# davide-coccomini/MINTIME-Multi-Identity-size-iNvariant-TIMEsformer-for-Video-Deepfake-Detection

Measured on AMD Instinct MI355X. Metric: clips/sec (8-frame, 2-identity, 224^2 crops) fwd+bwd, higher is better.
Workload: dtype f32; 1 GPU; config 3: EfficientNet-B0 + SizeInvariantTimeSformer(dim 512, depth 9, heads 8), B=32/GPU, 8 frames, 2 identities (identity-masked), 224x224 crops, random-init seeded weights (restored before every step), train-mode BN + drop-connect 0.2, step = fwd + BCE loss + bwd + SGD(lr .01, wd 1e-4); global_batch=32, frames=8, parallelism=dp1

## Files before the change

mintime-multi-identity-size-invariant-timesformer-for-video-deepfake-detection_amd/csrc/common.hpp:

```cpp
#pragma once
#include <hip/hip_runtime.h>
#include <stdio.h>
#include <stdarg.h>
#include <stdlib.h>
#include <map>
#include <mutex>
#include <utility>

namespace mt {

inline char* err_buf() {
  static thread_local char buf[512] = {0};
  return buf;
}

inline int fail(int code, const char* fmt, ...) {
  va_list ap;
  va_start(ap, fmt);
  vsnprintf(err_buf(), 512, fmt, ap);
  va_end(ap);
  return code;
}

inline int env_int(const char* name, int dflt) {
  const char* e = getenv(name);
  return e ? atoi(e) : dflt;
}
inline bool env_set(const char* name) { return getenv(name) != nullptr; }

inline int cur_device() {
  int d = 0;
  (void)hipGetDevice(&d);
  return d & 15;
}

inline hipError_t ensure_dynamic_lds(const void* kernel, size_t bytes) {
  if (bytes <= 48 * 1024) return hipSuccess;
  static std::mutex mu;
  static std::map<std::pair<const void*, int>, size_t> raised;
  int dev = 0;
  (void)hipGetDevice(&dev);
  std::lock_guard<std::mutex> g(mu);
  size_t& r = raised[std::make_pair(kernel, dev)];
  if (bytes <= r) return hipSuccess;
  const hipError_t e = hipFuncSetAttribute(kernel, hipFuncAttributeMaxDynamicSharedMemorySize, (int)bytes);
  if (e == hipSuccess) r = bytes;
  return e;
}

inline int check_launch(const char* what) {
  hipError_t e = hipGetLastError();
  if (e != hipSuccess) return fail(-2, "%s: launch failed: %s", what, hipGetErrorString(e));
  return 0;
}

int stem_wgrad_mfma(const float* du, const float* z, const float* kabc, const void* x, int x_is_u8, float* dw, int N, int H, int W,
                    int Ho, int Wo, int pad0, hipStream_t st);

enum { MT_ERR_ARG = -1, MT_ERR_LAUNCH = -2, MT_ERR_UNSUPPORTED = -3 };

int matmul_precision();

__device__ __forceinline__ void stat_add(double* p, int64_t limb, float v) {
  if (limb == 0) {
    atomicAdd(p, (double)v);
    return;
  }
  const float t = truncf(v);
  atomicAdd(reinterpret_cast<unsigned long long*>(p), (unsigned long long)(long long)t);
  atomicAdd(reinterpret_cast<unsigned long long*>(p + limb), (unsigned long long)__float2ll_rn((v - t) * 17592186044416.0f));
}
__device__ __forceinline__ double stat_get(const double* p, int64_t limb) {
  if (limb == 0) return *p;
  const long long hi = *reinterpret_cast<const long long*>(p), lo = *reinterpret_cast<const long long*>(p + limb);
  return (double)hi + (double)lo * 5.684341886080801486968994140625e-14;
}
__host__ __device__ __forceinline__ int stat_slots(int slots) { return slots < 0 ? -slots : (slots > 0 ? slots : 1); }
__host__ __device__ __forceinline__ int64_t stat_limb(int slots, int C) { return slots < 0 ? (int64_t)(-slots) * 2 * C : 0; }

__device__ __forceinline__ void xcd_chunk_tile(int chunks, int& chunk, int64_t& tile0, int64_t& stride) {
  const int xcd = blockIdx.x & 7, j = blockIdx.x >> 3;
  chunk = j % chunks;
  tile0 = (int64_t)(j / chunks) * 8 + xcd;
  stride = (int64_t)((gridDim.x >> 3) / chunks) * 8;
}

__device__ __forceinline__ void tile_nyx(int64_t tile, int ty_n, int tx_n, int& n, int& ty, int& tx) {
  const unsigned t = (unsigned)tile, t2 = t / (unsigned)tx_n;
  tx = (int)(t - t2 * (unsigned)tx_n);
  const unsigned nn = t2 / (unsigned)ty_n;
  ty = (int)(t2 - nn * (unsigned)ty_n);
  n = (int)nn;
}

__device__ __forceinline__ int64_t div_rows(int64_t r, int hw) {
  return (r >> 32) ? r / hw : (int64_t)((unsigned)r / (unsigned)hw);
}

struct FastDiv {
  uint32_t mul;
  int sh;
  __device__ __forceinline__ int div(int n) const { return mul ? (int)(__umulhi((uint32_t)n, mul) >> sh) : n; }
};
inline FastDiv fast_div_of(int d) {
  FastDiv f{0u, 0};
  if (d <= 1) return f;
  int l = 0;
  while (((int64_t)1 << l) < d) ++l;
  f.mul = (uint32_t)((((uint64_t)1 << (31 + l)) / (uint64_t)d) + 1);
  f.sh = l - 1;
  return f;
}

inline unsigned xcd_chunk_grid(int chunks, int64_t ntiles, int target_blocks) {
  if (ntiles >= ((int64_t)1 << 31)) return 0;
  int64_t per_xcd = target_blocks / (8 * chunks);
  const int64_t need = (ntiles + 7) / 8;
  if (per_xcd > need) per_xcd = need;
  if (per_xcd < 1) per_xcd = 1;
  return (unsigned)(8 * chunks * per_xcd);
}


__device__ __forceinline__ void lds_barrier() { asm volatile("s_waitcnt lgkmcnt(0)\n\ts_barrier" ::: "memory"); }

}
```

mintime-multi-identity-size-invariant-timesformer-for-video-deepfake-detection_amd/csrc/effnet_bwd.hip:

```cpp
#include "../../include/mintime_hip.h"
#include "common.hpp"
#include <type_traits>
#include "rc.hpp"
#include "det.hpp"
#include <stdlib.h>

using namespace mt;

namespace {

__device__ __forceinline__ float sigmoidf_(float x) { return __builtin_amdgcn_rcpf(1.0f + __expf(-x)); }
__device__ __forceinline__ float swishf_(float x) { return x * sigmoidf_(x); }
__device__ __forceinline__ float dswishf_(float u) { const float s = sigmoidf_(u); return s * (1.0f + u * (1.0f - s)); }

__device__ __forceinline__ float4 f4(float a, float b, float c, float d) { return make_float4(a, b, c, d); }
__device__ __forceinline__ float4 ld4(const float* p) { return *reinterpret_cast<const float4*>(p); }
__device__ __forceinline__ void st4(float* p, float4 v) { *reinterpret_cast<float4*>(p) = v; }
__device__ __forceinline__ float4 fma4(float4 a, float4 b, float4 c) {
  return f4(fmaf(a.x, b.x, c.x), fmaf(a.y, b.y, c.y), fmaf(a.z, b.z, c.z), fmaf(a.w, b.w, c.w));
}
__device__ __forceinline__ float4 mul4(float4 a, float4 b) { return f4(a.x * b.x, a.y * b.y, a.z * b.z, a.w * b.w); }
__device__ __forceinline__ float4 add4(float4 a, float4 b) { return f4(a.x + b.x, a.y + b.y, a.z + b.z, a.w + b.w); }

template <int ACT>
// ... 298 lines not shown
  constexpr int P = S == 1 ? (K - 1) / 2 : (K - 2) / 2;
  constexpr int CQN = CC / 4;
  constexpr int IH = (T - 1) * S + K;
  constexpr int IWP = IH | 1;
  constexpr int PS = (256 / CQN) / K;
  extern __shared__ __attribute__((aligned(16))) float lds[];
  float* a_t = lds;
  float* dz_t = lds + IH * IWP * CC;
  const int tid = threadIdx.x;
  const int cq = tid % CQN, r = tid / CQN;
  const int kh = r % K, ps = r / K;
  const bool worker = ps < PS;
  int chunk_id; int64_t tile0, tile_stride;
  xcd_chunk_tile(C / CC, chunk_id, tile0, tile_stride);
  const int c0 = chunk_id * CC;
  const int ty_n = (Ho + T - 1) / T, tx_n = (Wo + T - 1) / T;
  const int64_t ntiles = (int64_t)N * ty_n * tx_n;

  const float4 ka = ld4(kabc + c0 + cq * 4), kb = ld4(kabc + C + c0 + cq * 4), kc = ld4(kabc + 2 * C + c0 + cq * 4);
  const int lane = tid & 63;
  const int f_q = RC ? (lane >> 4) : cq, f_slot = RC ? ((tid >> 6) * 16 + (lane & 15)) : tid / CQN;
  const float4 sc = ld4(scale_in + c0 + f_q * 4), sh = ld4(shift_in + c0 + f_q * 4);
  constexpr int RCW = RC ? RC : 8;
  RcFrag<RCW> wfrag;
  if constexpr (RC > 0) rc_load<RCW>(wfrag, we + (int64_t)(c0 + (lane & 15)) * RC, lane);

  float4 acc[K];
#pragma unroll
  for (int i = 0; i < K; ++i) acc[i] = f4(0, 0, 0, 0);

  constexpr int NSL = 256 / CQN;
  constexpr int NL = (IH * IH + NSL - 1) / NSL, ND = (T * T + NSL - 1) / NSL;
  static_assert(NL <= 32 && ND <= 32, "validity masks are 32 bits");
  const int slot = tid / CQN;
  float4 pre[RC ? 1 : NL], pdu[ND], pz[ND];
  RcFrag<RCW> ypre[RC ? NL : 1];
  unsigned pre_ok = 0, pd_ok = 0;
  auto fetch = [&](int64_t tile) {
    int n, ty, tx;
    tile_nyx(tile, ty_n, tx_n, n, ty, tx);
    const int oh0 = ty * T, ow0 = tx * T;
    const int ih0 = oh0 * S - P, iw0 = ow0 * S - P;
    const float* img = RC ? zin + (int64_t)n * H * W * RC : zin + (int64_t)n * H * W * C + c0 + cq * 4;
    pre_ok = 0; pd_ok = 0;
#pragma unroll
    for (int i = 0; i < NL; ++i) {
      const int pix = f_slot + i * NSL;
      const int iy = pix / IH, ix = pix - iy * IH;
      const int ih = ih0 + iy, iw = iw0 + ix;
      if (pix < IH * IH && ih >= 0 && ih < H && iw >= 0 && iw < W) pre_ok |= 1u << i;
      const int64_t poff = (int64_t)min(max(ih, 0), H - 1) * W + min(max(iw, 0), W - 1);
      if constexpr (RC > 0) rc_load<RCW>(ypre[i], img + poff * RC, lane);
      else pre[i] = ld4(img + poff * C);
    }
    const int64_t obase = (int64_t)n * Ho * Wo * C + c0 + cq * 4;
#pragma unroll
    for (int i = 0; i < ND; ++i) {
      const int pix = slot + i * NSL;
      const int oy = pix / T, ox = pix - oy * T;
      const int oh = oh0 + oy, ow = ow0 + ox;
      if (pix < T * T && oh < Ho && ow < Wo) pd_ok |= 1u << i;
      const int64_t off = obase + ((int64_t)min(oh, Ho - 1) * Wo + min(ow, Wo - 1)) * C;
      pdu[i] = ld4(du + off);
      pz[i] = ld4(z + off);
    }
  };
  int64_t tile = tile0;
  if (tile < ntiles) fetch(tile);
  for (; tile < ntiles; tile += tile_stride) {
    __syncthreads();
#pragma unroll
    for (int i = 0; i < NL; ++i) {
      const int pix = f_slot + i * NSL;
      float4 zraw;
      if constexpr (RC > 0) zraw = rc_mma<RCW>(wfrag, ypre[i]);
      else zraw = pre[i];
      if (pix < IH * IH) {
        const int iy = pix / IH, ix = pix - iy * IH;
        const float4 v = act4<ACT>(fma4(zraw, sc, sh));
        const bool ok = (pre_ok >> i) & 1u;
        st4(a_t + (iy * IWP + ix) * CC + f_q * 4, f4(ok ? v.x : 0.f, ok ? v.y : 0.f, ok ? v.z : 0.f, ok ? v.w : 0.f));
      }
    }
#pragma unroll
    for (int i = 0; i < ND; ++i) {
      const int pix = slot + i * NSL;
      if (pix < T * T) {
        const float4 v = fma4(ka, pdu[i], fma4(kb, pz[i], kc));
        const bool ok = (pd_ok >> i) & 1u;
        st4(dz_t + pix * CC + cq * 4, f4(ok ? v.x : 0.f, ok ? v.y : 0.f, ok ? v.z : 0.f, ok ? v.w : 0.f));
      }
    }
    __syncthreads();
    if (tile + tile_stride < ntiles) fetch(tile + tile_stride);
    if (worker) {
      for (int p = ps; p < T * T; p += PS) {
        const int oy = p / T, ox = p - oy * T;
        const float4 d = ld4(dz_t + p * CC + cq * 4);
        const float* arow = a_t + ((oy * S + kh) * IWP + ox * S) * CC + cq * 4;
#pragma unroll
        for (int kw = 0; kw < K; ++kw) acc[kw] = fma4(d, ld4(arow + kw * CC), acc[kw]);
      }
    }
  }
  __syncthreads();
  float* red = lds;
  if (worker) {
#pragma unroll
    for (int kw = 0; kw < K; ++kw) st4(red + (((ps * K + kh) * CQN + cq) * K + kw) * 4, acc[kw]);
  }
  __syncthreads();
  if (tid < K * CQN * K) {
    const int kw = tid % K, q = (tid / K) % CQN, khh = tid / (CQN * K);
    float4 t = f4(0, 0, 0, 0);
    for (int g = 0; g < PS; ++g) t = add4(t, ld4(red + (((g * K + khh) * CQN + q) * K + kw) * 4));
    const int c = c0 + q * 4, tp = khh * K + kw;
    if (det.vals) {
      const int rk = (int)tile0, jb = q * 4 * K * K + tp;
      det_put(det, chunk_id, rk, jb, t.x); det_put(det, chunk_id, rk, jb + K * K, t.y);
      det_put(det, chunk_id, rk, jb + 2 * K * K, t.z); det_put(det, chunk_id, rk, jb + 3 * K * K, t.w);
      if (rk == 0 && tid == 0) det_base(det, chunk_id, (int64_t)c0 * K * K);
    } else {
      atomicAdd(dw + (c + 0) * K * K + tp, t.x); atomicAdd(dw + (c + 1) * K * K + tp, t.y);
      atomicAdd(dw + (c + 2) * K * K + tp, t.z); atomicAdd(dw + (c + 3) * K * K + tp, t.w);
    }
  }
}

template <int K, int S, int T, int ACT, int CC, int RC = 0>
int launch_dw_wgrad_tiled(const float* du, const float* z, const float* kabc, const float* zin, const float* scale_in,
                          const float* shift_in, float* dw, int N, int H, int W, int C, int Ho, int Wo, hipStream_t s,
                          const float* we = nullptr) {
  constexpr int IH = (T - 1) * S + K;
  constexpr int IWP = IH | 1;
  constexpr int CQN = CC / 4;
  constexpr int PS = (256 / CQN) / K;
  size_t lds = (size_t)(IH * IWP * CC + T * T * CC) * sizeof(float);
  const size_t red = (size_t)PS * K * CQN * K * 4 * sizeof(float);
  if (red > lds) lds = red;
  const int chunks = C / CC;
  const int64_t ntiles = (int64_t)N * ((Ho + T - 1) / T) * ((Wo + T - 1) / T);
  const unsigned bx = xcd_chunk_grid(chunks, ntiles, 4096);
  auto k = dwconv_wgrad_tiled_kernel<K, S, T, ACT, CC, RC>;
  if (lds > 48 * 1024) {
    hipError_t e = ensure_dynamic_lds(reinterpret_cast<const void*>(k), lds);
    if (e != hipSuccess) return fail(MT_ERR_LAUNCH, "mt_dwconv_bwd: cannot reserve %zu B of LDS: %s", lds, hipGetErrorString(e));
  }
  DetScope det(s, chunks, (int)((bx >> 3) / chunks) * 8, CC * K * K);
  hipLaunchKernelGGL(k, dim3(bx), dim3(256), lds, s, du, z, kabc, zin, scale_in, shift_in, dw, N, H, W, C, Ho, Wo, det.log, we);
  const int rc = check_launch("mt_dwconv_bwd(weight, tiled)");
  return rc ? rc : det.reduce_f32(dw);
}

thread_local int g_res_stride = 1;

template <int K, int S, int T, int ACT, int CC, bool WG = false, int RC = 0>
__global__ __launch_bounds__(256) void dwconv_dgrad_tiled_kernel(
    const float* __restrict__ du, const float* __restrict__ z, const float* __restrict__ kabc, const float* __restrict__ w,
    const float* __restrict__ zin, const float* __restrict__ scale_in, const float* __restrict__ shift_in,
    const float* __restrict__ mi_in, float* __restrict__ du_in, double* __restrict__ stats, int slots, int N, int H, int W,
    int C, int Ho, int Wo, const float* __restrict__ res_pre, const float* __restrict__ res_post, float* __restrict__ dw,
    int res_stride, const float* __restrict__ we) {
  static_assert(RC == 0 || CC == 16, "the recompute yields 16-channel chunks");
  constexpr int P = S == 1 ? (K - 1) / 2 : (K - 2) / 2;
  constexpr int CQN = CC / 4, NSLOT = 256 / CQN;
  constexpr int OT = (T - 1 + K - 1) / S + 2;
  constexpr int OTP = OT | 1;
  extern __shared__ __attribute__((aligned(16))) float lds[];
  const int tid = threadIdx.x;
  const int cq = tid % CQN, slot = tid / CQN;
  int chunk_id; int64_t tile0, tile_stride;
  xcd_chunk_tile(C / CC, chunk_id, tile0, tile_stride);
  const int c0 = chunk_id * CC;
  const int ty_n = (H + T - 1) / T, tx_n = (W + T - 1) / T;
  const int64_t ntiles = (int64_t)N * ty_n * tx_n;
  const int c = c0 + cq * 4;
  const float4 sc = ld4(scale_in + c), sh = ld4(shift_in + c);
  const float4 mean = mi_in ? ld4(mi_in + c) : f4(0, 0, 0, 0), istd = mi_in ? ld4(mi_in + C + c) : f4(0, 0, 0, 0);
  constexpr bool WLDS = K > 3 || S == 1;
  float* w_t = lds + OT * OTP * CC;
  float* z_t = w_t + (WLDS ? K * K * CC : 0);
  constexpr int RCW = RC ? RC : 8;
  constexpr int NLZ = (T * T + 63) / 64;
  const int lane = tid & 63;
  const int f_q = lane >> 4, f_slot = (tid >> 6) * 16 + (lane & 15);
  RcFrag<RCW> wfrag, ypre[RC ? NLZ : 1];
  if constexpr (RC > 0) rc_load<RCW>(wfrag, we + (int64_t)(c0 + (lane & 15)) * RC, lane);
  float4 wt[WLDS ? 1 : K * K];
  if constexpr (WLDS) {
    if (slot == 0)
      for (int i = 0; i < K * K; ++i)
        st4(w_t + i * CC + cq * 4, f4(w[(c + 0) * K * K + i], w[(c + 1) * K * K + i], w[(c + 2) * K * K + i], w[(c + 3) * K * K + i]));
  } else {
#pragma unroll
    for (int i = 0; i < K * K; ++i)
      wt[i] = f4(w[(c + 0) * K * K + i], w[(c + 1) * K * K + i], w[(c + 2) * K * K + i], w[(c + 3) * K * K + i]);
  }
  const float4 ka = ld4(kabc + c), kb = ld4(kabc + C + c), kc = ld4(kabc + 2 * C + c);
  float4 s1 = f4(0, 0, 0, 0), s2 = s1;
  float* a_t = z_t + (RC ? T * T * CC : 0);
  constexpr int PS2 = NSLOT / K;
  const int r2 = tid / CQN, kh2 = r2 % K, ps2 = r2 / K;
  float4 wacc[WG ? K : 1];
#pragma unroll
  for (int i = 0; i < (WG ? K : 1); ++i) wacc[i] = f4(0, 0, 0, 0);
  constexpr int ND = (OT * OT + NSLOT - 1) / NSLOT;
  static_assert(ND <= 32, "validity mask is 32 bits");
  float4 pdu[ND], pz[ND];
  unsigned pd_ok = 0;
  auto lows = [&](int64_t tile, int& n, int& ih0, int& iw0, int& oh_lo, int& ow_lo) {
    int ty, tx;
    tile_nyx(tile, ty_n, tx_n, n, ty, tx);
    ih0 = ty * T; iw0 = tx * T;
    const int nh = ih0 + P - (K - 1), nw = iw0 + P - (K - 1);
    oh_lo = nh >= 0 ? (nh + S - 1) / S : -((-nh) / S);
    ow_lo = nw >= 0 ? (nw + S - 1) / S : -((-nw) / S);
  };
  auto fetch = [&](int64_t tile) {
    int n, ih0, iw0, oh_lo, ow_lo;
    lows(tile, n, ih0, iw0, oh_lo, ow_lo);
    const int64_t obase = (int64_t)n * Ho * Wo * C + c;
    pd_ok = 0;
#pragma unroll
    for (int i = 0; i < ND; ++i) {
      const int pix = slot + i * NSLOT;
      const int oy = pix / OT, ox = pix - oy * OT;
      const int oh = oh_lo + oy, ow = ow_lo + ox;
      if (pix < OT * OT && oh >= 0 && oh < Ho && ow >= 0 && ow < Wo) pd_ok |= 1u << i;
      const int64_t off = obase + ((int64_t)min(max(oh, 0), Ho - 1) * Wo + min(max(ow, 0), Wo - 1)) * C;
      pdu[i] = ld4(du + off);
      pz[i] = ld4(z + off);
    }
    if constexpr (RC > 0) {
      const float* img = zin + (int64_t)n * H * W * RC;
#pragma unroll
      for (int i = 0; i < NLZ; ++i) {
        const int pix = f_slot + i * 64;
        const int iy = pix / T, ix = pix - iy * T;
        rc_load<RCW>(ypre[i], img + ((int64_t)min(ih0 + iy, H - 1) * W + min(iw0 + ix, W - 1)) * RC, lane);
      }
    }
  };
  int64_t tile = tile0;
  if (tile < ntiles) fetch(tile);
  for (; tile < ntiles; tile += tile_stride) {
    int n, ih0, iw0, oh_lo, ow_lo;
    lows(tile, n, ih0, iw0, oh_lo, ow_lo);
    __syncthreads();
#pragma unroll
    for (int i = 0; i < ND; ++i) {
      const int pix = slot + i * NSLOT;
      if (pix < OT * OT) {
        const int oy = pix / OT, ox = pix - oy * OT;
        const float4 v = fma4(ka, pdu[i], fma4(kb, pz[i], kc));
        const bool ok = (pd_ok >> i) & 1u;
        st4(lds + (oy * OTP + ox) * CC + cq * 4, f4(ok ? v.x : 0.f, ok ? v.y : 0.f, ok ? v.z : 0.f, ok ? v.w : 0.f));
      }
    }
    if constexpr (RC > 0) {
#pragma unroll
      for (int i = 0; i < NLZ; ++i) {
        const int pix = f_slot + i * 64;
        const float4 zq = rc_mma<RCW>(wfrag, ypre[i]);
        if (pix < T * T) st4(z_t + pix * CC + f_q * 4, zq);
      }
    }
    __syncthreads();
    if (tile + tile_stride < ntiles) fetch(tile + tile_stride);
#pragma unroll 1
    for (int p = slot; p < T * T; p += NSLOT) {
      const int iy = p / T, ix = p - iy * T;
      const int ih = ih0 + iy, iw = iw0 + ix;
      if constexpr (WG) {
        if (!(ih < H && iw < W)) st4(a_t + p * CC + cq * 4, f4(0, 0, 0, 0));
      }
      if (ih < H && iw < W) {
        float4 acc = f4(0, 0, 0, 0);
        const int64_t off = (((int64_t)n * H + ih) * W + iw) * C + c;
        float4 zz;
        if constexpr (RC > 0) zz = ld4(z_t + p * CC + cq * 4);
        else zz = ld4(zin + off);
        const float4 u = fma4(zz, sc, sh);
        if constexpr (WG) st4(a_t + p * CC + cq * 4, act4<ACT>(u));
        int wq = cq * 4;
        if constexpr (WLDS) asm volatile("" : "+v"(wq));
        auto tap = [&](int kh, int kw, int oy, int ox) {
          float4 ww;
          if constexpr (WLDS) ww = ld4(w_t + (kh * K + kw) * CC + wq);
          else ww = wt[kh * K + kw];
          acc = fma4(ld4(lds + (oy * OTP + ox) * CC + cq * 4), ww, acc);
        };
        if constexpr (S == 1) {
          const int oy0 = ih + P - oh_lo, ox0 = iw + P - ow_lo;
          if constexpr (WLDS) {
#pragma unroll 1
            for (int kh = 0; kh < K; ++kh) {
#pragma unroll
              for (int kw = 0; kw < K; ++kw) tap(kh, kw, oy0 - kh, ox0 - kw);
            }
          } else {
#pragma unroll
            for (int kh = 0; kh < K; ++kh) {
#pragma unroll
              for (int kw = 0; kw < K; ++kw) tap(kh, kw, oy0 - kh, ox0 - kw);
              __builtin_amdgcn_sched_barrier(0);
            }
          }
        } else {
          const int ph = (ih + P) & 1, pw = (iw + P) & 1;
          const int oyb = ((ih + P - ph) >> 1) - oh_lo, oxb = ((iw + P - pw) >> 1) - ow_lo;
          auto taps = [&](auto PH, auto PW) {
            constexpr int ph_ = decltype(PH)::value, pw_ = decltype(PW)::value;
#pragma unroll
            for (int kh = ph_; kh < K; kh += 2) {
#pragma unroll
              for (int kw = pw_; kw < K; kw += 2) tap(kh, kw, oyb - (kh - ph_) / 2, oxb - (kw - pw_) / 2);
              __builtin_amdgcn_sched_barrier(0);
            }
          };
          using I0 = std::integral_constant<int, 0>;
          using I1 = std::integral_constant<int, 1>;
          if (ph == 0) { if (pw == 0) taps(I0{}, I0{}); else taps(I0{}, I1{}); }
          else { if (pw == 0) taps(I1{}, I0{}); else taps(I1{}, I1{}); }
        }
        const bool r_on = res_stride == 1 || !((ih | iw) & 1);
        const int64_t roff = res_stride == 1 ? off : (((int64_t)n * ((H + 1) >> 1) + (ih >> 1)) * ((W + 1) >> 1) + (iw >> 1)) * C + c;
        if (res_pre && r_on) acc = add4(acc, ld4(res_pre + roff));
        float4 d = mul4(acc, dact4<ACT>(u));
        if (res_post && r_on) d = add4(d, ld4(res_post + roff));
        st4(du_in + off, d);
        const float4 xh = f4((zz.x - mean.x) * istd.x, (zz.y - mean.y) * istd.y, (zz.z - mean.z) * istd.z, (zz.w - mean.w) * istd.w);
        s1 = add4(s1, d);
        s2 = fma4(d, xh, s2);
      }
    }
    if constexpr (WG) {
      __syncthreads();
      if (ps2 < PS2) {
        const int ohb = ih0 + P - kh2;
#pragma unroll 1
        for (int p = ps2; p < T * T; p += PS2) {
          const int iy = p / T, ix = p - iy * T;
          const int ohn = ohb + iy;
          if (S == 2 && (ohn & 1)) continue;
          const float4 a = ld4(a_t + p * CC + cq * 4);
          const float* drow = lds + (((ohn >> (S - 1)) - oh_lo) * OTP) * CC + cq * 4;
          const int owb = iw0 + ix + P;
          if constexpr (S == 1) {
#pragma unroll
            for (int kw = 0; kw < K; ++kw) wacc[kw] = fma4(ld4(drow + (owb - kw - ow_lo) * CC), a, wacc[kw]);
          } else {
            const int pw = owb & 1, oxb = ((owb - pw) >> 1) - ow_lo;
            if (pw == 0) {
#pragma unroll
              for (int kw = 0; kw < K; kw += 2) wacc[kw] = fma4(ld4(drow + (oxb - kw / 2) * CC), a, wacc[kw]);
            } else {
#pragma unroll
              for (int kw = 1; kw < K; kw += 2) wacc[kw] = fma4(ld4(drow + (oxb - (kw - 1) / 2) * CC), a, wacc[kw]);
            }
          }
        }
      }
    }
  }
  if constexpr (WG) {
    __syncthreads();
    float* red = lds;
    if (ps2 < PS2) {
#pragma unroll
      for (int kw = 0; kw < K; ++kw) st4(red + (((ps2 * K + kh2) * CQN + cq) * K + kw) * 4, wacc[kw]);
    }
    __syncthreads();
    if (tid < K * CQN * K) {
      const int kw = tid % K, q = (tid / K) % CQN, khh = tid / (CQN * K);
      float4 t = f4(0, 0, 0, 0);
      for (int g = 0; g < PS2; ++g) t = add4(t, ld4(red + (((g * K + khh) * CQN + q) * K + kw) * 4));
      const int ch = c0 + q * 4, tp = khh * K + kw;
      atomicAdd(dw + (ch + 0) * K * K + tp, t.x); atomicAdd(dw + (ch + 1) * K * K + tp, t.y);
      atomicAdd(dw + (ch + 2) * K * K + tp, t.z); atomicAdd(dw + (ch + 3) * K * K + tp, t.w);
    }
  }
  if (!stats) return;
  __syncthreads();
  float* rr = lds + tid * 8;
  rr[0] = s1.x; rr[1] = s1.y; rr[2] = s1.z; rr[3] = s1.w; rr[4] = s2.x; rr[5] = s2.y; rr[6] = s2.z; rr[7] = s2.w;
  __syncthreads();
  if (tid < CQN * 8) {
    const int q = tid >> 3, e = tid & 7;
    float v = 0.f;
    for (int sl = 0; sl < NSLOT; ++sl) v += lds[(sl * CQN + q) * 8 + e];
    const int ch = c0 + q * 4 + (e & 3), which = e >> 2;
    stat_add(stats + ((int64_t)(blockIdx.x % stat_slots(slots)) * 2 + which) * C + ch, stat_limb(slots, C), v);
  }
}

template <int K, int S, int T, int ACT, int CC, bool WG = false, int RC = 0>
int launch_dw_dgrad_tiled(const float* du, const float* z, const float* kabc, const float* w, const float* zin,
                          const float* scale_in, const float* shift_in, const float* mi_in, float* du_in, double* stats, int slots,
                          int N, int H, int W, int C, int Ho, int Wo, const float* res_pre, const float* res_post, hipStream_t s,
                          float* dw = nullptr, const float* we = nullptr) {
  constexpr int OT = (T - 1 + K - 1) / S + 2;
  constexpr int OTP = OT | 1;
  constexpr int CQN = CC / 4, NSLOT = 256 / CQN;
  size_t lds = (size_t)(OT * OTP * CC + ((K > 3 || S == 1) ? K * K * CC : 0) + (RC ? T * T * CC : 0) + (WG ? T * T * CC : 0)) * sizeof(float);
  if (lds < 256 * 8 * sizeof(float)) lds = 256 * 8 * sizeof(float);
  if (WG && lds < (size_t)(NSLOT / K) * K * CQN * K * 4 * sizeof(float)) lds = (size_t)(NSLOT / K) * K * CQN * K * 4 * sizeof(float);
  const int chunks = C / CC;
  const int64_t ntiles = (int64_t)N * ((H + T - 1) / T) * ((W + T - 1) / T);
  const unsigned bx = xcd_chunk_grid(chunks, ntiles, WG ? 4096 : 8192);
  auto kfn = dwconv_dgrad_tiled_kernel<K, S, T, ACT, CC, WG, RC>;
  if (lds > 48 * 1024) {
    hipError_t e = ensure_dynamic_lds(reinterpret_cast<const void*>(kfn), lds);
    if (e != hipSuccess) return fail(MT_ERR_LAUNCH, "mt_dwconv_bwd: cannot reserve %zu B of LDS: %s", lds, hipGetErrorString(e));
  }
  hipLaunchKernelGGL(kfn, dim3(bx), dim3(256), lds, s, du, z, kabc, w, zin,
                     scale_in, shift_in, mi_in, du_in, stats, slots != 0 ? slots : 1, N, H, W, C, Ho, Wo, res_pre, res_post, dw,
                     g_res_stride, we);
  return check_launch(WG ? "mt_dwconv_bwd(data + weight, fused)" : "mt_dwconv_bwd(data, tiled)");
}

template <int K, int S, int ACT>
int launch_dw_bwd_tiled_any(const float* du, const float* z, const float* kabc, const float* w, const float* zin, const float* scale_in,
                            const float* shift_in, const float* mi_in, float* du_in, double* stats, int slots, float* dw, int N, int H,
                            int W, int C, int Ho, int Wo, int parts, const float* res_pre, const float* res_post, hipStream_t s) {
  int rc = 0;
  static const int t7_mask = env_int("MT_DW_T7", 0);
  const bool t14o = Ho >= 14 && !(t7_mask & 4), t14i = H >= 14 && !(t7_mask & 2);
  if (parts == 3) {
    if (C % 16 == 0) return t14i ? launch_dw_dgrad_tiled<K, S, 14, ACT, 16, true>(du, z, kabc, w, zin, scale_in, shift_in, mi_in, du_in, stats, slots, N, H, W, C, Ho, Wo, res_pre, res_post, s, dw)
                                 : launch_dw_dgrad_tiled<K, S, 7, ACT, 16, true>(du, z, kabc, w, zin, scale_in, shift_in, mi_in, du_in, stats, slots, N, H, W, C, Ho, Wo, res_pre, res_post, s, dw);
    return t14i ? launch_dw_dgrad_tiled<K, S, 14, ACT, 8, true>(du, z, kabc, w, zin, scale_in, shift_in, mi_in, du_in, stats, slots, N, H, W, C, Ho, Wo, res_pre, res_post, s, dw)
                : launch_dw_dgrad_tiled<K, S, 7, ACT, 8, true>(du, z, kabc, w, zin, scale_in, shift_in, mi_in, du_in, stats, slots, N, H, W, C, Ho, Wo, res_pre, res_post, s, dw);
  }
  if (parts & 1) {
    if (C % 16 == 0) rc = t14o ? launch_dw_wgrad_tiled<K, S, 14, ACT, 16>(du, z, kabc, zin, scale_in, shift_in, dw, N, H, W, C, Ho, Wo, s)
                               : launch_dw_wgrad_tiled<K, S, 7, ACT, 16>(du, z, kabc, zin, scale_in, shift_in, dw, N, H, W, C, Ho, Wo, s);
    else rc = t14o ? launch_dw_wgrad_tiled<K, S, 14, ACT, 8>(du, z, kabc, zin, scale_in, shift_in, dw, N, H, W, C, Ho, Wo, s)
                   : launch_dw_wgrad_tiled<K, S, 7, ACT, 8>(du, z, kabc, zin, scale_in, shift_in, dw, N, H, W, C, Ho, Wo, s);
    if (rc) return rc;
  }
  if (parts & 2) {
    if (C % 16 == 0) rc = t14i ? launch_dw_dgrad_tiled<K, S, 14, ACT, 16>(du, z, kabc, w, zin, scale_in, shift_in, mi_in, du_in, stats, slots, N, H, W, C, Ho, Wo, res_pre, res_post, s)
                               : launch_dw_dgrad_tiled<K, S, 7, ACT, 16>(du, z, kabc, w, zin, scale_in, shift_in, mi_in, du_in, stats, slots, N, H, W, C, Ho, Wo, res_pre, res_post, s);
    else rc = t14i ? launch_dw_dgrad_tiled<K, S, 14, ACT, 8>(du, z, kabc, w, zin, scale_in, shift_in, mi_in, du_in, stats, slots, N, H, W, C, Ho, Wo, res_pre, res_post, s)
                   : launch_dw_dgrad_tiled<K, S, 7, ACT, 8>(du, z, kabc, w, zin, scale_in, shift_in, mi_in, du_in, stats, slots, N, H, W, C, Ho, Wo, res_pre, res_post, s);
  }
  return rc;
}

__global__ __launch_bounds__(256) void stem_wgrad_kernel(const float* __restrict__ du, const float* __restrict__ z,
                                                         const float* __restrict__ kabc, const void* __restrict__ xv, int x_u8,
                                                         float* __restrict__ dw, int N, int H, int W, int Ho, int Wo, int pad0,
                                                         const DetLog det) {
  const float* x = reinterpret_cast<const float*>(xv);
  const uint8_t* xb = reinterpret_cast<const uint8_t*>(xv);
  constexpr int CO = 32, TP = 64, TAPS = 27;
  __shared__ float dzt[TP][CO + 1];
  __shared__ float xt[TP][TAPS + 1];
  const int tid = threadIdx.x;
  const int co = tid & 31, g = tid >> 5;
  const float ka = kabc[co], kb = kabc[CO + co], kc = kabc[2 * CO + co];
  float acc[4] = {0.f, 0.f, 0.f, 0.f};
  const int64_t total = (int64_t)N * Ho * Wo;
  const int64_t ntiles = (total + TP - 1) / TP;
  for (int64_t tile = blockIdx.x; tile < ntiles; tile += gridDim.x) {
    const int64_t p0 = tile * TP;
    __syncthreads();
    for (int i = tid; i < TP * CO; i += 256) {
      const int p = i >> 5, c2 = i & 31;
      const int64_t pix = p0 + p;
      float v = 0.f;
      if (pix < total) v = fmaf(kabc[c2], du[pix * CO + c2], fmaf(kabc[CO + c2], z[pix * CO + c2], kabc[2 * CO + c2]));
      dzt[p][c2] = v;
    }
    for (int i = tid; i < TP * TAPS; i += 256) {
      const int p = i / TAPS, tp = i - p * TAPS;
      const int ci = tp % 3, kk = tp / 3, kw = kk % 3, kh = kk / 3;
      const int64_t pix = p0 + p;
      float v = 0.f;
      if (pix < total) {
        const int ow = (int)(pix % Wo);
        const int64_t t = pix / Wo;
        const int oh = (int)(t % Ho), n = (int)(t / Ho);
        const int ih = oh * 2 + kh - pad0, iw = ow * 2 + kw - pad0;
        if (ih >= 0 && ih < H && iw >= 0 && iw < W) {
          const int64_t off = (((int64_t)n * H + ih) * W + iw) * 3 + ci;
          v = x_u8 ? (float)xb[off] : x[off];
        }
      }
      xt[p][tp] = v;
    }
    __syncthreads();
#pragma unroll 8
    for (int p = 0; p < TP; ++p) {
      const float d = dzt[p][co];
#pragma unroll
      for (int i = 0; i < 4; ++i) {
        const int tp = g + 8 * i;
        if (tp < TAPS) acc[i] = fmaf(d, xt[p][tp], acc[i]);
      }
    }
  }
  (void)ka; (void)kb; (void)kc;
#pragma unroll
  for (int i = 0; i < 4; ++i) {
    const int tp = g + 8 * i;
    if (tp < TAPS) {
      const int ci = tp % 3, kk = tp / 3, kw = kk % 3, kh = kk / 3;
      if (det.vals) det_put(det, 0, blockIdx.x, ((co * 3 + ci) * 3 + kh) * 3 + kw, acc[i]);
      else atomicAdd(dw + ((co * 3 + ci) * 3 + kh) * 3 + kw, acc[i]);
    }
  }
}

int pick_cqb(int CQ) {
  int best = 1;
  for (int d = 1; d <= 64 && d <= CQ; ++d)
    if (CQ % d == 0) best = d;
  return best;
}

template <int K, int S>
int launch_dw_bwd(const float* du, const float* z, const float* kabc, const float* w, const float* zin, const float* scale_in,
                  const float* shift_in, const float* mi_in, float* du_in, double* stats, int slots, float* dw, int N, int H,
                  int W, int C, int parts, int act, const float* res_pre, const float* res_post, hipStream_t s) {
  const int Ho = (H + S - 1) / S, Wo = (W + S - 1) / S;
  if (C % 8 != 0) return fail(MT_ERR_UNSUPPORTED, "mt_dwconv_bwd: channel count %d is not a multiple of 8", C);
  if (act == 1) return launch_dw_bwd_tiled_any<K, S, 1>(du, z, kabc, w, zin, scale_in, shift_in, mi_in, du_in, stats, slots, dw, N, H, W, C, Ho, Wo, parts, res_pre, res_post, s);
  if (act == 2) return launch_dw_bwd_tiled_any<K, S, 2>(du, z, kabc, w, zin, scale_in, shift_in, mi_in, du_in, stats, slots, dw, N, H, W, C, Ho, Wo, parts, res_pre, res_post, s);
  return launch_dw_bwd_tiled_any<K, S, 0>(du, z, kabc, w, zin, scale_in, shift_in, mi_in, du_in, stats, slots, dw, N, H, W, C, Ho, Wo, parts, res_pre, res_post, s);
}

}

extern "C" int mt_bn_act_bwd(const float* din, const float* z, const float* scale, const float* shift,
                             const float* mean_invstd, const float* gate, const float* dpool, const float* rowscale,
                             float* dout, double* stats, int slots, int64_t rows, int C, int hw, int act, void* stream) {
  if (!din || !z || !scale || !shift || !mean_invstd || !stats) return fail(MT_ERR_ARG, "mt_bn_act_bwd: null pointer");
  if ((gate == nullptr) != (dpool == nullptr)) return fail(MT_ERR_ARG, "mt_bn_act_bwd: gate and dpool go together");
  if (C & 3) return fail(MT_ERR_ARG, "mt_bn_act_bwd: C %% 4 != 0");
  const int CQ = C / 4, CQB = pick_cqb(CQ), PB = 256 / CQB;
  int64_t nb = (rows + PB - 1) / PB;
  const int64_t cap = 4096 / (CQ / CQB) > 0 ? 4096 / (CQ / CQB) : 1;
  if (nb > cap) nb = cap;
  hipLaunchKernelGGL(bn_act_bwd_kernel, dim3((unsigned)nb, CQ / CQB), dim3(CQB * PB), (size_t)PB * CQB * 8 * sizeof(float),
                     (hipStream_t)stream, din, z, scale, shift, mean_invstd, gate, dpool, rowscale, dout, stats,
                     slots != 0 ? slots : 1, rows, C, hw > 0 ? hw : 1, act, CQB, PB);
  return check_launch("mt_bn_act_bwd");
}

extern "C" int mt_bn_bwd_finalize(const double* stats, int slots, double count, const float* gamma, const float* mean_invstd,
                                  float* kabc, float* dgamma, float* dbeta, int C, int training, void* stream) {
  if (!stats || !gamma || !mean_invstd || !kabc) return fail(MT_ERR_ARG, "mt_bn_bwd_finalize: null pointer");
  hipLaunchKernelGGL(bn_bwd_finalize_kernel, dim3((C + 31) / 32), dim3(256), 0, (hipStream_t)stream, stats, slots, count, gamma,
                     mean_invstd, kabc, dgamma, dbeta, C, training);
  return check_launch("mt_bn_bwd_finalize");
}

static int se_adjoint(const float* dgate, const float* gate, const float* hidden, const float* w1, const float* w2, float* dpre2,
                      float* dhid, float* dpooled, float* scratch, int N, int C, int CS, hipStream_t s) {
  const int slabs = (C + SE_SLAB - 1) / SE_SLAB;
  hipLaunchKernelGGL(se_bwd_slab_kernel, dim3(N, slabs), dim3(256), (size_t)(SE_SLAB + SE_SLAB * (CS + 1)) * sizeof(float), s, dgate, gate,
                     w2, dpre2, scratch, C, CS);
  int rc = check_launch("mt_se_bwd(slab)");
  if (rc) return rc;
  hipLaunchKernelGGL(se_bwd_finish_kernel, dim3(N, (C + 255) / 256), dim3(256), (size_t)CS * sizeof(float), s, scratch, slabs, hidden, w1,
                     dhid, dpooled, C, CS);
  return check_launch("mt_se_bwd(finish)");
}

extern "C" int mt_se_scratch_floats(int N, int C, int CS) { return N * ((C + SE_SLAB - 1) / SE_SLAB) * CS; }

extern "C" int mt_se_bwd(const float* da, const float* z, const float* scale, const float* shift, const float* gate,
                         const float* hidden, const float* pooled, const float* w1, const float* w2, float* dgate,
                         float* dpre2, float* dhid, float* dpooled, float* dw1, float* db1, float* dw2, float* db2, int N,
                         int HW, int C, int CS, int parts_mask, float* scratch, void* stream) {
  if (((parts_mask & 1) && (!da || !z || !scale || !shift)) || !gate || !hidden || !pooled || !w1 || !w2 || !dgate || !dpre2 || !dhid ||
      !dpooled || !dw1 || !db1 || !dw2 || !db2 || ((parts_mask & 5) && !scratch))
    return fail(MT_ERR_ARG, "mt_se_bwd: null pointer");
  if (C & 3) return fail(MT_ERR_ARG, "mt_se_bwd: C %% 4 != 0");
  if (CS > CS_MAX) return fail(MT_ERR_UNSUPPORTED, "mt_se_bwd: squeeze width %d > %d", CS, CS_MAX);
  hipStream_t s = (hipStream_t)stream;
  const int CQ = C / 4, CQB = pick_cqb(CQ), PB = 256 / CQB;
  int rc = 0;
  if (parts_mask & 1) {
  int parts = 1;
  while ((int64_t)N * (CQ / CQB) * parts < 2048 && HW / (parts * 2) >= PB * 16) parts *= 2;
  if (det_enabled()) parts = 1;
  if (parts > 1 && hipMemsetAsync(dgate, 0, (size_t)N * C * sizeof(float), s) != hipSuccess)
    return fail(MT_ERR_LAUNCH, "mt_se_bwd: memset failed");
  hipLaunchKernelGGL(se_bwd_reduce_kernel, dim3(N, CQ / CQB, parts), dim3(CQB * PB), (size_t)PB * CQB * 4 * sizeof(float), s, da, z,
                     scale, shift, dgate, HW, C, CQB, PB);
  rc = check_launch("mt_se_bwd(reduce)");
  if (rc) return rc;
  rc = se_adjoint(dgate, gate, hidden, w1, w2, dpre2, dhid, dpooled, scratch, N, C, CS, s);
  if (rc) return rc;
  }
  if (parts_mask & 4) {
// ... 95 lines not shown
```

mintime-multi-identity-size-invariant-timesformer-for-video-deepfake-detection_amd/csrc/gemm_dma.hpp:

```cpp
#pragma once
#include "gemm_core.hpp"

#ifndef MT_DMA_FN_ALIGN
#define MT_DMA_FN_ALIGN 256
#endif
#ifndef MT_DMA_LOOP_ALIGN
#define MT_DMA_LOOP_ALIGN 0
#endif
#ifndef MT_DMA_ISSUE_MID
#define MT_DMA_ISSUE_MID 0
#endif
#ifndef MT_DMA_ABLATE
#define MT_DMA_ABLATE 0
#endif

namespace mt {

__device__ __forceinline__ void lds_dma16(const float* gsrc, unsigned lds_byte_addr) {
  unsigned keep;
  asm volatile("s_mov_b32 %0, m0\n\ts_mov_b32 m0, %2\n\ts_nop 0\n\tglobal_load_lds_dwordx4 %1, off\n\ts_mov_b32 m0, %0"
               : "=&s"(keep) : "v"(gsrc), "s"(lds_byte_addr) : "memory");
}

template <int N> __device__ __forceinline__ void wait_vmcnt() { asm volatile("s_waitcnt vmcnt(%0)" ::"n"(N) : "memory"); }

#define MT_STR2(x) #x
#define MT_STR(x) MT_STR2(x)

enum { MMA_F32 = 0, MMA_BF16X6 = 1, MMA_BF16X3 = 2 };
typedef __bf16 bf16x8_t __attribute__((ext_vector_type(8)));
typedef __bf16 bf16x2_t __attribute__((ext_vector_type(2)));
typedef float f32x2_t __attribute__((ext_vector_type(2)));

template <bool THREE>
__device__ __forceinline__ void split_bf16(const float (&lo)[4], const float (&hi)[4], bf16x8_t& x0, bf16x8_t& x1, bf16x8_t& x2) {
#pragma unroll
  for (int q = 0; q < 4; ++q) {
    const f32x2_t v = q < 2 ? f32x2_t{lo[2 * q], lo[2 * q + 1]} : f32x2_t{hi[2 * q - 4], hi[2 * q - 3]};
    const bf16x2_t a = __builtin_convertvector(v, bf16x2_t);
    const f32x2_t r = v - __builtin_convertvector(a, f32x2_t);
    const bf16x2_t b = __builtin_convertvector(r, bf16x2_t);
    x0[2 * q] = a[0]; x0[2 * q + 1] = a[1];
    x1[2 * q] = b[0]; x1[2 * q + 1] = b[1];
    if constexpr (THREE) {
      const f32x2_t t = r - __builtin_convertvector(b, f32x2_t);
      const bf16x2_t c = __builtin_convertvector(t, bf16x2_t);
      x2[2 * q] = c[0]; x2[2 * q + 1] = c[1];
    }
  }
}

template <int WAVES_M, int WAVES_N, int TM, int TN, int AL, int BL, int EPI, int BK, int STAGES, int MINW, int PRO = PRO_NONE,
          int MMA = MMA_F32>
__global__ __launch_bounds__(WAVES_M * WAVES_N * 64, MINW) __attribute__((aligned(MT_DMA_FN_ALIGN)))
void gemm_dma_kernel(const GemmArgs p) {
  static_assert(PRO == PRO_NONE || AL == LAYOUT_KCONTIG, "fragment-time prologues are implemented for k-contiguous A");
  static_assert(PRO == PRO_NONE || PRO == PRO_BN_SWISH_GATE || PRO == PRO_BN_BWD, "unsupported prologue");
  constexpr bool TWO_A = PRO == PRO_BN_BWD;
  constexpr int NW = WAVES_M * WAVES_N;
  constexpr int BM = WAVES_M * TM * 32;
  constexpr int BN = WAVES_N * TN * 32;
  constexpr int GPR = BK / 4;
  constexpr int SW_SHIFT = BK == 16 ? 2 : 1;
  constexpr int A_TILE = BM * BK, B_TILE = BN * BK;
  constexpr int STAGE = A_TILE * (TWO_A ? 2 : 1) + B_TILE;
  constexpr int A2_OFF = A_TILE + B_TILE;
  constexpr int A_INSTR = A_TILE / 256, B_INSTR = B_TILE / 256;
  static_assert(A_INSTR % NW == 0 && B_INSTR % NW == 0, "every wavefront must issue the same number of DMA instructions");
  constexpr int A_IPW = A_INSTR / NW, B_IPW = B_INSTR / NW, IPW = A_IPW * (TWO_A ? 2 : 1) + B_IPW;
  static_assert(BK == 16 || BK == 32, "BK must be 16 or 32");
  static_assert(STAGES >= 2 && STAGES <= 4, "2..4 stages");
  constexpr int NG = BK / 8;

  extern __shared__ __attribute__((aligned(16))) float smem_dma[];
  const unsigned lds_base = (unsigned)(uintptr_t)(__attribute__((address_space(3))) float*)smem_dma;

  const int tid = threadIdx.x;
  const int lane = tid & 63;
  const int wave = __builtin_amdgcn_readfirstlane(tid >> 6);
  const int wm = wave / WAVES_N;
  const int wn = wave % WAVES_N;

  int mt_, nt_;
  if (!tile_coords<BM, BN>(p, mt_, nt_)) return;
  const int m0 = mt_ * BM;
  const int n0 = nt_ * BN;

  int k_begin = 0, k_end = p.K;
  if (p.k_chunk > 0) {
    k_begin = blockIdx.y * p.k_chunk;
    k_end = min(p.K, k_begin + p.k_chunk);
    if (k_begin >= k_end) return;
  }
  const int nk = (k_end - k_begin) / BK;

  const float* a_src[A_IPW];
  const float* b_src[B_IPW];
  int64_t a2_delta = 0;
  int a_k[A_IPW], b_k[B_IPW];
#pragma unroll
  for (int j = 0; j < A_IPW; ++j) {
    const int gi = (wave * A_IPW + j) * 64 + lane;
    if constexpr (AL == LAYOUT_KCONTIG) {
      const int row = gi / GPR, slot = gi % GPR;
      const int kq = slot ^ ((row >> SW_SHIFT) & (GPR - 1));
      int m = m0 + row;
      m = m < p.M ? m : p.M - 1;
      a_src[j] = p.A + map_row(p.a_map, m) * p.lda + k_begin + kq * 4;
      a_k[j] = 0;
      if constexpr (TWO_A) a2_delta = p.A2 - p.A;
    } else {
      constexpr int CPR = BM / 4;
      const int kk = gi / CPR, cq = gi % CPR;
      int m = m0 + cq * 4;
      m = m < p.M ? m : p.M - 4;
      a_src[j] = p.A + m;
      a_k[j] = kk;
    }
  }
#pragma unroll
  for (int j = 0; j < B_IPW; ++j) {
    const int gi = (wave * B_IPW + j) * 64 + lane;
    if constexpr (BL == LAYOUT_KCONTIG) {
      const int row = gi / GPR, slot = gi % GPR;
      const int kq = slot ^ ((row >> SW_SHIFT) & (GPR - 1));
      int n;
      if constexpr (EPI == EPI_GEGLU) {
        static_assert(EPI != EPI_GEGLU || TN == 2, "GEGLU wants TN == 2");
        const int w = row / 64, sel = (row >> 5) & 1, c = row & 31;
        const int jj = (n0 >> 1) + w * 32 + c;
        n = jj < p.n_half ? sel * p.n_half + jj : 0;
      } else {
        n = n0 + row;
        n = n < p.N ? n : p.N - 1;
      }
      b_src[j] = p.B + (int64_t)n * p.ldb + k_begin + kq * 4;
      b_k[j] = 0;
    } else {
      constexpr int CPR = BN / 4;
      const int kk = gi / CPR, cq = gi % CPR;
      int n = n0 + cq * 4;
      n = n < p.N ? n : p.N - 4;
      b_src[j] = p.B + n;
      b_k[j] = kk;
    }
  }

  auto issue = [&](int kt) {
    if (MT_DMA_ABLATE & 1) return;
    const unsigned st = lds_base + (unsigned)((kt % STAGES) * STAGE * 4);
    const int k0 = k_begin + kt * BK;
#pragma unroll
    for (int j = 0; j < A_IPW; ++j) {
      const float* src;
      if constexpr (AL == LAYOUT_KCONTIG) src = a_src[j] + kt * BK;
      else src = a_src[j] + map_row(p.a_map, k0 + a_k[j]) * p.lda;
      lds_dma16(src, st + (unsigned)((wave * A_IPW + j) * 1024));
      if constexpr (TWO_A) lds_dma16(src + a2_delta, st + (unsigned)(A2_OFF * 4 + (wave * A_IPW + j) * 1024));
    }
#pragma unroll
    for (int j = 0; j < B_IPW; ++j) {
      const float* src;
      if constexpr (BL == LAYOUT_KCONTIG) src = b_src[j] + kt * BK;
      else src = b_src[j] + map_row(p.b_map, k0 + b_k[j]) * p.ldb;
      lds_dma16(src, st + (unsigned)(A_TILE * 4 + (wave * B_IPW + j) * 1024));
    }
  };

  f32x16 acc[TM][TN];
#pragma unroll
  for (int i = 0; i < TM; ++i)
#pragma unroll
    for (int j = 0; j < TN; ++j)
#pragma unroll
      for (int r = 0; r < 16; ++r) acc[i][j][r] = 0.f;

  const int khalf = lane >> 5;
// ... 155 lines not shown
```

Baseline: 730.7 clips/s.

## Double-buffer depthwise dgrad input tiles into LDS via global-to-LDS DMA prefetch

Adds a staged variant of the depthwise-conv dgrad tiled kernel. It uses global_load_lds_dwordx4 to copy the next tile's input activations into a double-buffered LDS region while the current tile is computed. The inner loop then reads activations from LDS instead of global memory. The variant is selected per kernel size, stride and fused/unfused form through an env bitmask; the default enables only the fused 3x3 stride-2 case. It costs extra LDS per block, which can lower occupancy, and adds a vmcnt wait before each barrier.

```diff
diff --git a/mintime-multi-identity-size-invariant-timesformer-for-video-deepfake-detection_amd/csrc/common.hpp b/mintime-multi-identity-size-invariant-timesformer-for-video-deepfake-detection_amd/csrc/common.hpp
--- a/mintime-multi-identity-size-invariant-timesformer-for-video-deepfake-detection_amd/csrc/common.hpp
+++ b/mintime-multi-identity-size-invariant-timesformer-for-video-deepfake-detection_amd/csrc/common.hpp
@@ -124,4 +124,12 @@
 
 __device__ __forceinline__ void lds_barrier() { asm volatile("s_waitcnt lgkmcnt(0)\n\ts_barrier" ::: "memory"); }
 
+__device__ __forceinline__ void lds_dma16(const float* gsrc, unsigned lds_byte_addr) {
+  unsigned keep;
+  asm volatile("s_mov_b32 %0, m0\n\ts_mov_b32 m0, %2\n\ts_nop 0\n\tglobal_load_lds_dwordx4 %1, off\n\ts_mov_b32 m0, %0"
+               : "=&s"(keep) : "v"(gsrc), "s"(lds_byte_addr) : "memory");
 }
+
+template <int N> __device__ __forceinline__ void wait_vmcnt() { asm volatile("s_waitcnt vmcnt(%0)" ::"n"(N) : "memory"); }
+
+}
diff --git a/mintime-multi-identity-size-invariant-timesformer-for-video-deepfake-detection_amd/csrc/effnet_bwd.hip b/mintime-multi-identity-size-invariant-timesformer-for-video-deepfake-detection_amd/csrc/effnet_bwd.hip
--- a/mintime-multi-identity-size-invariant-timesformer-for-video-deepfake-detection_amd/csrc/effnet_bwd.hip
+++ b/mintime-multi-identity-size-invariant-timesformer-for-video-deepfake-detection_amd/csrc/effnet_bwd.hip
@@ -474,9 +474,11 @@
   return rc ? rc : det.reduce_f32(dw);
 }
 
+constexpr int dw_stage_instr(int T, int CC) { return (T * T * CC * 4 + 1023) / 1024; }
+
 thread_local int g_res_stride = 1;
 
-template <int K, int S, int T, int ACT, int CC, bool WG = false, int RC = 0>
+template <int K, int S, int T, int ACT, int CC, bool WG = false, int RC = 0, bool ST = false>
 __global__ __launch_bounds__(256) void dwconv_dgrad_tiled_kernel(
     const float* __restrict__ du, const float* __restrict__ z, const float* __restrict__ kabc, const float* __restrict__ w,
     const float* __restrict__ zin, const float* __restrict__ scale_in, const float* __restrict__ shift_in,
@@ -484,6 +486,7 @@
     int C, int Ho, int Wo, const float* __restrict__ res_pre, const float* __restrict__ res_post, float* __restrict__ dw,
     int res_stride, const float* __restrict__ we) {
   static_assert(RC == 0 || CC == 16, "the recompute yields 16-channel chunks");
+  static_assert(!ST || RC == 0, "the staged form is the plain form's; the recompute form has its own LDS tile");
   constexpr int P = S == 1 ? (K - 1) / 2 : (K - 2) / 2;
   constexpr int CQN = CC / 4, NSLOT = 256 / CQN;
   constexpr int OT = (T - 1 + K - 1) / S + 2;
@@ -526,6 +529,11 @@
   float4 wacc[WG ? K : 1];
 #pragma unroll
   for (int i = 0; i < (WG ? K : 1); ++i) wacc[i] = f4(0, 0, 0, 0);
+  constexpr int ZI = dw_stage_instr(T, CC);
+  float* z_r = a_t + (WG ? T * T * CC : 0);
+  const unsigned z_r_addr = (unsigned)(uintptr_t)(__attribute__((address_space(3))) float*)z_r;
+  const int wave = __builtin_amdgcn_readfirstlane(tid >> 6);
+  int rs = 0;
   constexpr int ND = (OT * OT + NSLOT - 1) / NSLOT;
   static_assert(ND <= 32, "validity mask is 32 bits");
   float4 pdu[ND], pz[ND];
@@ -563,8 +571,28 @@
       }
     }
   };
+  auto stage = [&](int64_t tile, int to) {
+    int ty, tx, n;
+    tile_nyx(tile, ty_n, tx_n, n, ty, tx);
+    const int ih0 = ty * T, iw0 = tx * T;
+    const float* img = zin + (int64_t)n * H * W * C + c;
+    int ln = lane;
+    asm volatile("" : "+v"(ln));
+#pragma unroll
+    for (int j = 0; j < (ZI + 3) / 4; ++j) {
+      const int q = wave + 4 * j;
+      if (q < ZI) {
+        const int p = min(q * (64 / CQN) + ln / CQN, T * T - 1);
+        const int iy = p / T, ix = p - iy * T;
+        lds_dma16(img + ((int64_t)min(ih0 + iy, H - 1) * W + min(iw0 + ix, W - 1)) * C, z_r_addr + (unsigned)((to * ZI + q) * 1024));
+      }
+    }
+  };
   int64_t tile = tile0;
-  if (tile < ntiles) fetch(tile);
+  if (tile < ntiles) {
+    if constexpr (ST) stage(tile, 0);
+    fetch(tile);
+  }
   for (; tile < ntiles; tile += tile_stride) {
     int n, ih0, iw0, oh_lo, ow_lo;
     lows(tile, n, ih0, iw0, oh_lo, ow_lo);
@@ -587,8 +615,17 @@
         if (pix < T * T) st4(z_t + pix * CC + f_q * 4, zq);
       }
     }
+    if constexpr (ST) wait_vmcnt<0>();
     __syncthreads();
-    if (tile + tile_stride < ntiles) fetch(tile + tile_stride);
+    if (tile + tile_stride < ntiles) {
+      if constexpr (ST) {
+        stage(tile + tile_stride, rs ^ 1);
+        __builtin_amdgcn_sched_barrier(0);
+      }
+      fetch(tile + tile_stride);
+    }
+    const float* z_c = z_r + rs * (ZI * 256);
+    rs ^= 1;
 #pragma unroll 1
     for (int p = slot; p < T * T; p += NSLOT) {
       const int iy = p / T, ix = p - iy * T;
@@ -601,6 +638,7 @@
         const int64_t off = (((int64_t)n * H + ih) * W + iw) * C + c;
         float4 zz;
         if constexpr (RC > 0) zz = ld4(z_t + p * CC + cq * 4);
+        else if constexpr (ST) zz = ld4(z_c + p * CC + cq * 4);
         else zz = ld4(zin + off);
         const float4 u = fma4(zz, sc, sh);
         if constexpr (WG) st4(a_t + p * CC + cq * 4, act4<ACT>(u));
@@ -716,7 +754,7 @@
   }
 }
 
-template <int K, int S, int T, int ACT, int CC, bool WG = false, int RC = 0>
+template <int K, int S, int T, int ACT, int CC, bool WG = false, int RC = 0, bool ST = false>
 int launch_dw_dgrad_tiled(const float* du, const float* z, const float* kabc, const float* w, const float* zin,
                           const float* scale_in, const float* shift_in, const float* mi_in, float* du_in, double* stats, int slots,
                           int N, int H, int W, int C, int Ho, int Wo, const float* res_pre, const float* res_post, hipStream_t s,
@@ -725,12 +763,13 @@
   constexpr int OTP = OT | 1;
   constexpr int CQN = CC / 4, NSLOT = 256 / CQN;
   size_t lds = (size_t)(OT * OTP * CC + ((K > 3 || S == 1) ? K * K * CC : 0) + (RC ? T * T * CC : 0) + (WG ? T * T * CC : 0)) * sizeof(float);
+  if (ST) lds += (size_t)2 * dw_stage_instr(T, CC) * 1024;
   if (lds < 256 * 8 * sizeof(float)) lds = 256 * 8 * sizeof(float);
   if (WG && lds < (size_t)(NSLOT / K) * K * CQN * K * 4 * sizeof(float)) lds = (size_t)(NSLOT / K) * K * CQN * K * 4 * sizeof(float);
   const int chunks = C / CC;
   const int64_t ntiles = (int64_t)N * ((H + T - 1) / T) * ((W + T - 1) / T);
   const unsigned bx = xcd_chunk_grid(chunks, ntiles, WG ? 4096 : 8192);
-  auto kfn = dwconv_dgrad_tiled_kernel<K, S, T, ACT, CC, WG, RC>;
+  auto kfn = dwconv_dgrad_tiled_kernel<K, S, T, ACT, CC, WG, RC, ST>;
   if (lds > 48 * 1024) {
     hipError_t e = ensure_dynamic_lds(reinterpret_cast<const void*>(kfn), lds);
     if (e != hipSuccess) return fail(MT_ERR_LAUNCH, "mt_dwconv_bwd: cannot reserve %zu B of LDS: %s", lds, hipGetErrorString(e));
@@ -739,6 +778,24 @@
                      scale_in, shift_in, mi_in, du_in, stats, slots != 0 ? slots : 1, N, H, W, C, Ho, Wo, res_pre, res_post, dw,
                      g_res_stride, we);
   return check_launch(WG ? "mt_dwconv_bwd(data + weight, fused)" : "mt_dwconv_bwd(data, tiled)");
+}
+
+constexpr int DW_STAGED_DEFAULT = 32;
+template <int K, int S>
+bool dw_staged(bool fused) {
+  const int bit = ((K == 5 ? 4 : 1) << (S == 2 ? 1 : 0)) << (fused ? 4 : 0);
+  return (env_int("MT_DW_STAGED", DW_STAGED_DEFAULT) & bit) != 0;
+}
+
+template <int K, int S, int ACT, bool WG, bool ST>
+int launch_dw_dgrad_form(bool t14, const float* du, const float* z, const float* kabc, const float* w, const float* zin,
+                         const float* scale_in, const float* shift_in, const float* mi_in, float* du_in, double* stats, int slots,
+                         int N, int H, int W, int C, int Ho, int Wo, const float* res_pre, const float* res_post, hipStream_t s,
+                         float* dw) {
+  if (C % 16 == 0) return t14 ? launch_dw_dgrad_tiled<K, S, 14, ACT, 16, WG, 0, ST>(du, z, kabc, w, zin, scale_in, shift_in, mi_in, du_in, stats, slots, N, H, W, C, Ho, Wo, res_pre, res_post, s, dw)
+                              : launch_dw_dgrad_tiled<K, S, 7, ACT, 16, WG, 0, ST>(du, z, kabc, w, zin, scale_in, shift_in, mi_in, du_in, stats, slots, N, H, W, C, Ho, Wo, res_pre, res_post, s, dw);
+  return t14 ? launch_dw_dgrad_tiled<K, S, 14, ACT, 8, WG, 0, ST>(du, z, kabc, w, zin, scale_in, shift_in, mi_in, du_in, stats, slots, N, H, W, C, Ho, Wo, res_pre, res_post, s, dw)
+             : launch_dw_dgrad_tiled<K, S, 7, ACT, 8, WG, 0, ST>(du, z, kabc, w, zin, scale_in, shift_in, mi_in, du_in, stats, slots, N, H, W, C, Ho, Wo, res_pre, res_post, s, dw);
 }
 
 template <int K, int S, int ACT>
@@ -749,10 +806,9 @@
   static const int t7_mask = env_int("MT_DW_T7", 0);
   const bool t14o = Ho >= 14 && !(t7_mask & 4), t14i = H >= 14 && !(t7_mask & 2);
   if (parts == 3) {
-    if (C % 16 == 0) return t14i ? launch_dw_dgrad_tiled<K, S, 14, ACT, 16, true>(du, z, kabc, w, zin, scale_in, shift_in, mi_in, du_in, stats, slots, N, H, W, C, Ho, Wo, res_pre, res_post, s, dw)
-                                 : launch_dw_dgrad_tiled<K, S, 7, ACT, 16, true>(du, z, kabc, w, zin, scale_in, shift_in, mi_in, du_in, stats, slots, N, H, W, C, Ho, Wo, res_pre, res_post, s, dw);
-    return t14i ? launch_dw_dgrad_tiled<K, S, 14, ACT, 8, true>(du, z, kabc, w, zin, scale_in, shift_in, mi_in, du_in, stats, slots, N, H, W, C, Ho, Wo, res_pre, res_post, s, dw)
-                : launch_dw_dgrad_tiled<K, S, 7, ACT, 8, true>(du, z, kabc, w, zin, scale_in, shift_in, mi_in, du_in, stats, slots, N, H, W, C, Ho, Wo, res_pre, res_post, s, dw);
+    return dw_staged<K, S>(true)
+        ? launch_dw_dgrad_form<K, S, ACT, true, true>(t14i, du, z, kabc, w, zin, scale_in, shift_in, mi_in, du_in, stats, slots, N, H, W, C, Ho, Wo, res_pre, res_post, s, dw)
+        : launch_dw_dgrad_form<K, S, ACT, true, false>(t14i, du, z, kabc, w, zin, scale_in, shift_in, mi_in, du_in, stats, slots, N, H, W, C, Ho, Wo, res_pre, res_post, s, dw);
   }
   if (parts & 1) {
     if (C % 16 == 0) rc = t14o ? launch_dw_wgrad_tiled<K, S, 14, ACT, 16>(du, z, kabc, zin, scale_in, shift_in, dw, N, H, W, C, Ho, Wo, s)
@@ -762,10 +818,9 @@
     if (rc) return rc;
   }
   if (parts & 2) {
-    if (C % 16 == 0) rc = t14i ? launch_dw_dgrad_tiled<K, S, 14, ACT, 16>(du, z, kabc, w, zin, scale_in, shift_in, mi_in, du_in, stats, slots, N, H, W, C, Ho, Wo, res_pre, res_post, s)
-                               : launch_dw_dgrad_tiled<K, S, 7, ACT, 16>(du, z, kabc, w, zin, scale_in, shift_in, mi_in, du_in, stats, slots, N, H, W, C, Ho, Wo, res_pre, res_post, s);
-    else rc = t14i ? launch_dw_dgrad_tiled<K, S, 14, ACT, 8>(du, z, kabc, w, zin, scale_in, shift_in, mi_in, du_in, stats, slots, N, H, W, C, Ho, Wo, res_pre, res_post, s)
-                   : launch_dw_dgrad_tiled<K, S, 7, ACT, 8>(du, z, kabc, w, zin, scale_in, shift_in, mi_in, du_in, stats, slots, N, H, W, C, Ho, Wo, res_pre, res_post, s);
+    rc = dw_staged<K, S>(false)
+        ? launch_dw_dgrad_form<K, S, ACT, false, true>(t14i, du, z, kabc, w, zin, scale_in, shift_in, mi_in, du_in, stats, slots, N, H, W, C, Ho, Wo, res_pre, res_post, s, nullptr)
+        : launch_dw_dgrad_form<K, S, ACT, false, false>(t14i, du, z, kabc, w, zin, scale_in, shift_in, mi_in, du_in, stats, slots, N, H, W, C, Ho, Wo, res_pre, res_post, s, nullptr);
   }
   return rc;
 }
diff --git a/mintime-multi-identity-size-invariant-timesformer-for-video-deepfake-detection_amd/csrc/gemm_dma.hpp b/mintime-multi-identity-size-invariant-timesformer-for-video-deepfake-detection_amd/csrc/gemm_dma.hpp
--- a/mintime-multi-identity-size-invariant-timesformer-for-video-deepfake-detection_amd/csrc/gemm_dma.hpp
+++ b/mintime-multi-identity-size-invariant-timesformer-for-video-deepfake-detection_amd/csrc/gemm_dma.hpp
@@ -16,13 +16,6 @@
 
 namespace mt {
 
-__device__ __forceinline__ void lds_dma16(const float* gsrc, unsigned lds_byte_addr) {
-  unsigned keep;
-  asm volatile("s_mov_b32 %0, m0\n\ts_mov_b32 m0, %2\n\ts_nop 0\n\tglobal_load_lds_dwordx4 %1, off\n\ts_mov_b32 m0, %0"
-               : "=&s"(keep) : "v"(gsrc), "s"(lds_byte_addr) : "memory");
-}
-
-template <int N> __device__ __forceinline__ void wait_vmcnt() { asm volatile("s_waitcnt vmcnt(%0)" ::"n"(N) : "memory"); }
 
 #define MT_STR2(x) #x
 #define MT_STR(x) MT_STR2(x)
```

Result: no change. 734.5 clips/s, median of 6 (+0.5%).
